# elasota/ConvectionKernels

Hardware: AMD Instinct MI355X
Metric: bc7_encode_default_plan_throughput (higher is better)
Workload: dtype f32+u16; 1 GPU; EncodeBC7, BC7EncodingPlan() + Options(), 4096x4096 SplitMix64 random RGBA, seed 2, 1048576 blocks resident in HBM (BASELINE configs[1]); blocks=1048576, exchange=none, search=exact branch-and-bound (output bit-identical)

## Files before the change

### convectionkernels_amd/csrc/bc7_kernel.hip

```cpp
#include <hip/hip_runtime.h>
#include <stdint.h>
#include <float.h>
#include <type_traits>
#include <stdlib.h>

#include "cvtt_device.h"

constexpr int kMaxPTRefine = 2;
constexpr float kBoundGrid16 = 2000.0f, kBoundLimit16 = 2040.0f;
constexpr float kBoundGrid8 = 124.0f, kBoundLimit8 = 127.0f;
#ifndef CVTT_GRID8_RGBA
#define CVTT_GRID8_RGBA true
#endif
#ifndef CVTT_GRID8_RGB
#define CVTT_GRID8_RGB true
#endif
#ifndef CVTT_BC7_WAVES
#define CVTT_BC7_WAVES 4
#endif
#ifndef CVTT_BC7_WAVES_SLOW
#define CVTT_BC7_WAVES_SLOW 4
#endif
#ifndef CVTT_EIG_ITERS
#define CVTT_EIG_ITERS 6
#endif

#include "cvtt_kernel_common.h"

#ifndef CVTT_SPEC_1
#define CVTT_SPEC_1 32
#define CVTT_SPEC_2 16
#define CVTT_SPEC_4 8
#define CVTT_SPEC_8 4
#endif
#ifndef CVTT_SPEC_16
#define CVTT_SPEC_16 2
#endif
#ifndef CVTT_FILTER_STRIKES
#define CVTT_FILTER_STRIKES 2
#endif
#ifndef CVTT_SHARP_COST4
#define CVTT_SHARP_COST4 64
#endif
#ifndef CVTT_SHARP_COST8
#define CVTT_SHARP_COST8 20
#endif
#ifndef CVTT_PEND_MIN
#define CVTT_PEND_MIN 20
#endif

#ifdef CVTT_BC7_PROFILE
__device__ unsigned long long g_bc7Prof[48];
__device__ unsigned long long g_bc7Dup[8];
__device__ unsigned long long g_bc7Stage[6][8];
__device__ unsigned long long g_bc7Stage2[6][8];
extern "C" int cvttmi_bc7_stage_read(unsigned long long *out)
{
    unsigned long long zero[48] = {0};
    if (hipMemcpyFromSymbol(out, HIP_SYMBOL(g_bc7Stage), sizeof(zero)) != hipSuccess) return -1;
    if (hipMemcpyToSymbol(HIP_SYMBOL(g_bc7Stage), zero, sizeof(zero)) != hipSuccess) return -1;
    if (hipMemcpyFromSymbol(out + 48, HIP_SYMBOL(g_bc7Stage2), sizeof(zero)) != hipSuccess) return -1;
    if (hipMemcpyToSymbol(HIP_SYMBOL(g_bc7Stage2), zero, sizeof(zero)) != hipSuccess) return -1;
    return 0;
}
#define PROF_STAGE(stage, slot, n) { const unsigned long long v_ = (unsigned long long)(n); if (threadIdx.x == 0 && v_) atomicAdd(&g_bc7Stage[stage][slot], v_); }
#define PROF_STAGE_LANES(stage, slot, pred) { const unsigned long long v_ = (unsigned long long)__popcll(__ballot(pred)); if (threadIdx.x == 0 && v_) atomicAdd(&g_bc7Stage[stage][slot], v_); }
#define PROF_STAGE2(stage, slot, n) { const unsigned long long v_ = (unsigned long long)(n); if (threadIdx.x == 0 && v_) atomicAdd(&g_bc7Stage2[stage][slot], v_); }
extern "C" int cvttmi_bc7_dup_read(unsigned long long *out)
{
    unsigned long long zero[8] = {0};
    if (hipMemcpyFromSymbol(out, HIP_SYMBOL(g_bc7Dup), sizeof(zero)) != hipSuccess) return -1;
    if (hipMemcpyToSymbol(HIP_SYMBOL(g_bc7Dup), zero, sizeof(zero)) != hipSuccess) return -1;
    return 0;
}
#define PROF_DECL unsigned long long profT = __builtin_readcyclecounter(); unsigned long long profAcc[16] = {0, 0, 0, 0, 0, 0, 0, 0, 0, 0, 0, 0, 0, 0, 0, 0}; unsigned long long profCnt[8] = {0, 0, 0, 0, 0, 0, 0, 0};
#define PROF_MARK(slot) { const unsigned long long now = __builtin_readcyclecounter(); profAcc[slot] += now - profT; profT = now; }
#define PROF_FLUSH if (threadIdx.x == 0) { unsigned long long tot = 0; for (int i = 0; i < 16; i++) { atomicAdd(&g_bc7Prof[i], profAcc[i]); tot += profAcc[i]; } \
    int bucket = 63 - __builtin_clzll(tot | 1ull) - 12; bucket = bucket < 0 ? 0 : (bucket > 15 ? 15 : bucket); atomicAdd(&g_bc7Prof[16 + bucket], 1ull); \
    } { unsigned long long wsum[8]; for (int i = 0; i < 8; i++) { unsigned long long v = profCnt[i]; if (i >= 4) { for (int st = 1; st < 64; st <<= 1) v += __shfl_xor(v, st); } wsum[i] = v; } \
    if (threadIdx.x == 0) { for (int i = 0; i < 8; i++) atomicAdd(&g_bc7Prof[32 + i], wsum[i]); \
    const unsigned long long passes = profCnt[2] / 64ull; int pb = 63 - __builtin_clzll(passes | 1ull); pb = pb > 7 ? 7 : pb; atomicAdd(&g_bc7Prof[40 + pb], 1ull); } }
#define PROF_COUNT(slot, n) { profCnt[slot] += (unsigned long long)(n); }
extern "C" int cvttmi_bc7_prof_read(unsigned long long *out)
{
    unsigned long long zero[48] = {0};
    if (hipMemcpyFromSymbol(out, HIP_SYMBOL(g_bc7Prof), sizeof(zero)) != hipSuccess) return -1;
    if (hipMemcpyToSymbol(HIP_SYMBOL(g_bc7Prof), zero, sizeof(zero)) != hipSuccess) return -1;
    return 0;
}
#else
#define PROF_DECL
#define PROF_MARK(slot)
#define PROF_COUNT(slot, n)
#define PROF_FLUSH
#define PROF_STAGE(stage, slot, n)
#define PROF_STAGE2(stage, slot, n)
#define PROF_STAGE_LANES(stage, slot, pred)
#endif

#ifdef CVTT_BC7_DEBUG
__device__ float g_bc7Dbg[2048];
__device__ unsigned g_bc7DbgBlock = 0xffffffffu;
extern "C" int cvttmi_bc7_debug_set(unsigned block)
{
    return hipMemcpyToSymbol(HIP_SYMBOL(g_bc7DbgBlock), &block, sizeof(block)) == hipSuccess ? 0 : -1;
}
extern "C" int cvttmi_bc7_debug_read(float *out)
{
    return hipMemcpyFromSymbol(out, HIP_SYMBOL(g_bc7Dbg), sizeof(float) * 2048) == hipSuccess ? 0 : -1;
}
#endif

namespace
{
__device__ __forceinline__ int quantizeNoP(int v, int bits) { return ((v << bits) - v + (127 + (1 << (7 - bits)))) >> 8; }
__device__ __forceinline__ int quantizeP(int v, int bits, int p)
{
    const int addend = p ? ((1 << (8 - bits)) - 1) : 255;
    const int q = ((v << (bits + 1)) - v + addend) >> 9;
    return (q << 1) | p;
}
__device__ __forceinline__ int unquantize(int v, int bits)
{
    const int t = v << (8 - bits);
    return t | (t >> bits);
}

struct ModeDesc
{
    int mode;
    int indexBits;
    int numP;
    int quantBits;
    int unquantBits;
};

__device__ __forceinline__ void compressEndpoints(const ModeDesc &md, int (&ep)[2][4], int pIter, bool isRGB)
{
    const int nch = isRGB ? 3 : 4;
#pragma unroll
    for (int j = 0; j < 2; j++)
    {
        const int p = (md.numP == 4) ? ((pIter >> j) & 1) : (pIter & 1);
#pragma unroll
        for (int ch = 0; ch < 4; ch++)
        {
            if (ch < nch)
            {
                int v = ep[j][ch];
                v = (md.numP == 1) ? quantizeNoP(v, md.quantBits) : quantizeP(v, md.quantBits, p);
                if (md.unquantBits)
                    v = unquantize(v, md.unquantBits);
                ep[j][ch] = v;
            }
        }
        if (isRGB)
            ep[j][3] = 255;
    }
}

struct ShapeBest
{
    float err;
    u32 ep0, ep1;
    u32 idxLo, idxHi;
};

__device__ __forceinline__ u32 packEP(const int (&e)[4])
{
    return (u32)e[0] | ((u32)e[1] << 8) | ((u32)e[2] << 16) | ((u32)e[3] << 24);
}

__device__ __forceinline__ void quadArgminBroadcast(ShapeBest &b, int lane)
{
    int who = lane & 3;
    float err = b.err;
// ... 1235 lines not shown
        for (int a = 0; a < 4; a++)
#pragma unroll
            for (int b = 0; b <= a; b++)
                r.p[tri(a, b)] = (int)__builtin_amdgcn_udot4(m[a], P[b][g], (u32)r.p[tri(a, b)], false);
    }
}

__device__ __forceinline__ void rawSumsSub(RawSums &d, const RawSums &a)
{
    d.n -= a.n;
#pragma unroll
    for (int i = 0; i < 4; i++)
        d.s[i] -= a.s[i];
#pragma unroll
    for (int i = 0; i < 10; i++)
        d.p[i] -= a.p[i];
}

template <int N>
__device__ __forceinline__ float subsetBoundFull(const RawSums &r, const float (&w)[4], float delta)
{
    if (r.n < 2)
        return 0.0f;
    const float n = (float)r.n;
    const float inv = __builtin_amdgcn_rcpf(n);
    Moments<N> m;
#pragma unroll
    for (int a = 0; a < N; a++)
#pragma unroll
        for (int b = 0; b <= a; b++)
        {
            const int v = __mul24(r.n, r.p[tri(a, b)]) - __mul24(r.s[a], r.s[b]);
            m.cov[tri(a, b)] = (((float)v * inv) * w[a]) * w[b];
        }
    return shapeErrorLowerBound<N>(m, n, delta);
}

__device__ __forceinline__ void topEigenvector(const float (&M)[10], float (&e)[4])
{
    int k = 0;
    float d = M[tri(0, 0)];
#pragma unroll
    for (int i = 1; i < 4; i++)
        if (M[tri(i, i)] > d)
        {
            d = M[tri(i, i)];
            k = i;
        }
    float v[4];
#pragma unroll
    for (int i = 0; i < 4; i++)
        v[i] = (k == 0) ? M[tri(i, 0)] : (k == 1) ? M[tri(i, 1)] : (k == 2) ? M[tri(i, 2)] : M[tri(i, 3)];
    for (int it = 0; it < CVTT_EIG_ITERS; it++)
    {
        float nv[4];
        float big = 0.0f;
#pragma unroll
        for (int r = 0; r < 4; r++)
        {
            float a = M[tri(r, 0)] * v[0];
#pragma unroll
            for (int c = 1; c < 4; c++)
                a = __fmaf_rn(M[tri(r, c)], v[c], a);
            nv[r] = a;
            big = fmaxf(big, fabsf(a));
        }
        const float sc = (big > 0.0f) ? __builtin_amdgcn_rcpf(big) : 0.0f;
#pragma unroll
        for (int r = 0; r < 4; r++)
            v[r] = nv[r] * sc;
    }
    float len = v[0] * v[0];
#pragma unroll
    for (int i = 1; i < 4; i++)
        len = __fmaf_rn(v[i], v[i], len);
    const bool ok = len > 1e-12f && len < 1e12f;
    const float inv = ok ? __builtin_amdgcn_rsqf(len) : 0.0f;
    e[0] = ok ? v[0] * inv : 1.0f;
#pragma unroll
    for (int i = 1; i < 4; i++)
        e[i] = v[i] * inv;
}

template <int N>
__device__ __forceinline__ float subsetBoundSharp(const u32 *lp, u32 mask, const float (&w)[4], float delta, float wSq, bool fourLevels)
{
    RawSums r;
    {
        asm volatile("" : "+v"(lp));
        u32 px[16], CM[4][4];
#pragma unroll
        for (int i = 0; i < 4; i++)
        {
            const uint4 v = *reinterpret_cast<const uint4 *>(lp + 4 * i);
            px[4 * i + 0] = v.x;
            px[4 * i + 1] = v.y;
            px[4 * i + 2] = v.z;
            px[4 * i + 3] = v.w;
        }
        channelMajor(px, CM);
        maskedRawSumsCM(CM, mask, r);
    }
    if (r.n < 2)
        return 0.0f;
    const float n = (float)r.n;
    const float inv = __builtin_amdgcn_rcpf(n);
    Moments<N> m;
#pragma unroll
    for (int a = 0; a < N; a++)
#pragma unroll
        for (int b = 0; b <= a; b++)
        {
            const int v = __mul24(r.n, r.p[tri(a, b)]) - __mul24(r.s[a], r.s[b]);
            m.cov[tri(a, b)] = (((float)v * inv) * w[a]) * w[b];
        }
    float rTrue;
    const float cur = shapeErrorLowerBound<N>(m, n, delta, &rTrue);
    if (r.n < 3 || !(rTrue >= 0.0f))
        return cur;
    float T = 0.0f;
#pragma unroll
    for (int i = 0; i < N; i++)
        T += m.cov[tri(i, i)];
    float e[4];
    {
        float M[10];
#pragma unroll
        for (int i = 0; i < 10; i++)
            M[i] = (N == 4 || i < 6) ? m.cov[i < N * (N + 1) / 2 ? i : 0] : 0.0f;
        topEigenvector(M, e);
    }
    float L = 0.0f, Sd[N];
#pragma unroll
    for (int a = 0; a < N; a++)
    {
        float acc = 0.0f;
#pragma unroll
        for (int b = 0; b < N; b++)
            acc = __fmaf_rn(m.cov[a >= b ? tri(a, b) : tri(b, a)], e[b], acc);
        Sd[a] = acc;
        L = __fmaf_rn(e[a], acc, L);
    }
    float rho2 = 0.0f, aMax = 0.0f, aSum = 0.0f;
#pragma unroll
    for (int a = 0; a < N; a++)
    {
        const float t = Sd[a] - L * e[a];
        rho2 = __fmaf_rn(t, t, rho2);
        const float ac = fabsf(e[a]) * w[a];
        aMax = fmaxf(aMax, ac);
        aSum += ac;
    }
    const float eta = 1e-5f * T;
    const float Llo = fmaxf(L - eta, 0.0f);
    const float Rlo = fmaxf(T - L - eta, 0.0f);
    const float sqrtRhi = __builtin_amdgcn_sqrtf(fmaxf(T - L, 0.0f) + eta) * 1.000001f;
    const float rhoHi = __builtin_amdgcn_sqrtf(rho2) * 1.000001f + eta;
    const float W2 = wSq * 1.000001f;
    const float md = fmaxf(2.0f * aMax - aSum, 0.0f) * 0.99999f;
    const float perp = __builtin_amdgcn_sqrtf(fmaxf(W2 - md * md, 0.0f)) * 1.000001f;

    float sqrtQ = 0.0f;
    constexpr int kMaxN = 13;
    if (fourLevels && r.n > 4 && r.n <= kMaxN)
    {
        float g[4];
// ... 37 lines not shown
        float D2[kMaxN + 1], D3[kMaxN + 1];
        D2[0] = D3[0] = 0.0f;
        {
            float su = 0.0f, sq = 0.0f;
#pragma unroll
            for (int j = 1; j <= kMaxN; j++)
            {
                su += t[j - 1];
                sq = __fmaf_rn(t[j - 1], t[j - 1], sq);
                D2[j] = D3[j] = __fmaf_rn(-su * su, kRcp[j], sq);
            }
        }
        float fin = D3[kMaxN];
        {
            float su0 = 0.0f, sq0 = 0.0f;
#pragma unroll
            for (int i = 1; i < kMaxN; i++)
            {
                su0 += t[i - 1];
                sq0 = __fmaf_rn(t[i - 1], t[i - 1], sq0);
                const float d1 = __fmaf_rn(-su0 * su0, kRcp[i], sq0);
                const float d2 = D2[i], d3 = D3[i];
                float su = 0.0f, sq = 0.0f;
#pragma unroll
                for (int j = i + 1; j <= kMaxN; j++)
                {
                    su += t[j - 1];
                    sq = __fmaf_rn(t[j - 1], t[j - 1], sq);
                    const float cst = __fmaf_rn(-su * su, kRcp[j - i], sq);
                    D2[j] = fminf(D2[j], d1 + cst);
                    D3[j] = fminf(D3[j], d2 + cst);
                }
                const float m = (float)(cnt - i);
                const float last = __fmaf_rn(-su * su, __builtin_amdgcn_rcpf(m), sq);
                fin = (i < cnt) ? fminf(fin, d3 + last) : fin;
            }
        }
        const float Q = fmaxf(fin - 2e-5f * range * range, 0.0f);
        sqrtQ = fmaxf(__builtin_amdgcn_sqrtf(fmaxf(Q * 0.9999f, 0.0f)) - 2e-3f, 0.0f);
    }

    constexpr int kIntervals = 20;
    constexpr float kB0sq[20] = {0.0f, 0.0001f, 0.0004f, 0.0009f, 0.0016f, 0.003025f, 0.0049f, 0.007225f, 0.01f, 0.015625f, 0.0225f, 0.030625f, 0.04f, 0.0625f, 0.09f, 0.140625f, 0.2025f, 0.3025f, 0.49f, 0.7225f};
    constexpr float kB1sq[20] = {0.0001f, 0.0004f, 0.0009f, 0.0016f, 0.003025f, 0.0049f, 0.007225f, 0.01f, 0.015625f, 0.0225f, 0.030625f, 0.04f, 0.0625f, 0.09f, 0.140625f, 0.2025f, 0.3025f, 0.49f, 0.7225f, 1.0f};
    constexpr float kB1[20] = {0.01f, 0.02f, 0.03f, 0.04f, 0.055f, 0.07f, 0.085f, 0.1f, 0.125f, 0.15f, 0.175f, 0.2f, 0.25f, 0.3f, 0.375f, 0.45f, 0.55f, 0.7f, 0.85f, 1.0f};
    constexpr float kA1[20] = {0.999948f, 0.999798f, 0.9995479f, 0.9991977f, 0.9984844f, 0.997545f, 0.996379f, 0.9949854f, 0.9921548f, 0.988684f, 0.9845665f, 0.9797939f, 0.9682439f, 0.9539373f, 0.927023f, 0.8930268f, 0.835163f, 0.7141414f, 0.5267816f, 0.0f};
    constexpr float kCross[20] = {0.00999952f, 0.01999604f, 0.02998656f, 0.03996807f, 0.05491686f, 0.06982843f, 0.08469255f, 0.09949894f, 0.1240198f, 0.1483032f, 0.1722998f, 0.1959596f, 0.2420619f, 0.2861823f, 0.347635f, 0.4018637f, 0.4593415f, 0.499901f, 0.500001f, 0.4477662f};
    float best = FLT_MAX;
#pragma unroll
    for (int j = 0; j < kIntervals; j++)
    {
        const float e0 = __fmaf_rn(kB0sq[j], Llo - Rlo, Rlo), e1 = __fmaf_rn(kB1sq[j], Llo - Rlo, Rlo);
        float base = fminf(e0, e1) * 0.999999f - 2.0f * kCross[j] * rhoHi;
        base = fmaxf(base, rTrue);
        const float qd = fmaxf(kA1[j] * sqrtQ - kB1[j] * sqrtRhi, 0.0f);
        const float G = __fmaf_rn(qd, qd, base);
        const float inner = fmaxf(kA1[j] * md - kB1[j] * perp, 0.0f);
        const float s2 = 0.25f * (W2 - inner * inner) * 1.000001f;
        float v = 0.0f;
        if (G > 4.0001f * n * s2)
            v = G - 2.0f * __builtin_amdgcn_sqrtf(s2 * n * G) * 1.000001f;
        best = fminf(best, v);
    }
    return fmaxf(cur, best * 0.9999f);
}

__device__ __forceinline__ int dot4s(u32 a, u32 b, int acc) { return __builtin_amdgcn_sdot4((int)a, (int)b, acc, false); }
template <bool G8>
struct Proj2D
{
    u32 U[G8 ? 4 : 8], V[G8 ? 4 : 8];
    int tU, tV, tUU, tVV, tUV;
};

template <bool G8>
__device__ __forceinline__ void makeProjection(const u32 (&pix)[16], const BlockScatter &bs, const CvttBc7Args &A,
                                               bool use4, float scale, Proj2D<G8> &P)
{
    float M[10];
#pragma unroll
    for (int i = 0; i < 10; i++)
        M[i] = (use4 || i < 6) ? bs.S[i] : 0.0f;
    float e1[4], e2[4];
    topEigenvector(M, e1);
    {
        float Me[4];
#pragma unroll
        for (int r = 0; r < 4; r++)
        {
            float a = M[tri(r, 0)] * e1[0];
#pragma unroll
            for (int c = 1; c < 4; c++)
                a = __fmaf_rn(M[tri(r, c)], e1[c], a);
            Me[r] = a;
        }
        float lam = Me[0] * e1[0];
#pragma unroll
        for (int r = 1; r < 4; r++)
            lam = __fmaf_rn(Me[r], e1[r], lam);
#pragma unroll
        for (int r = 0; r < 4; r++)
#pragma unroll
            for (int c = 0; c <= r; c++)
                M[tri(r, c)] = __fmaf_rn(-lam * e1[r], e1[c], M[tri(r, c)]);
    }
    topEigenvector(M, e2);
    {
        float d = e2[0] * e1[0];
#pragma unroll
        for (int i = 1; i < 4; i++)
            d = __fmaf_rn(e2[i], e1[i], d);
        float len = 0.0f;
#pragma unroll
        for (int i = 0; i < 4; i++)
        {
            e2[i] = __fmaf_rn(-d, e1[i], e2[i]);
            len = __fmaf_rn(e2[i], e2[i], len);
        }
        if (!(len > 1e-4f))
        {
            int k = 0;
            float small = fabsf(e1[0]);
#pragma unroll
            for (int i = 1; i < 4; i++)
                if ((use4 || i < 3) && fabsf(e1[i]) < small)
                {
                    small = fabsf(e1[i]);
                    k = i;
                }
            const float ek = (k == 0) ? e1[0] : (k == 1) ? e1[1] : (k == 2) ? e1[2] : e1[3];
            len = 0.0f;
#pragma unroll
            for (int i = 0; i < 4; i++)
            {
                e2[i] = ((i == k) ? 1.0f : 0.0f) - ek * e1[i];
                len = __fmaf_rn(e2[i], e2[i], len);
            }
        }
        const float inv = __builtin_amdgcn_rsqf(len);
#pragma unroll
        for (int i = 0; i < 4; i++)
            e2[i] *= inv;
    }
    if (!use4)
        e1[3] = e2[3] = 0.0f;

    float g1[4], g2[4];
    float o1 = 0.0f, o2 = 0.0f;
#pragma unroll
    for (int ch = 0; ch < 4; ch++)
    {
        g1[ch] = e1[ch] * A.w[ch] * scale;
        g2[ch] = e2[ch] * A.w[ch] * scale;
        o1 = __fmaf_rn(e1[ch] * scale, bs.meanW[ch], o1);
        o2 = __fmaf_rn(e2[ch] * scale, bs.meanW[ch], o2);
    }
    P.tU = P.tV = P.tUU = P.tVV = P.tUV = 0;
    if constexpr (G8)
    {
    int tid = (int)__builtin_amdgcn_mbcnt_hi(~0u, __builtin_amdgcn_mbcnt_lo(~0u, 0u));
    asm volatile("" : "+v"(tid));
    const int c = tid & 3;
    u32 myU = 0, myV = 0;
    {
        u32 ub = 0, vb = 0;
#pragma unroll
        for (int h = 0; h < 4; h++)
        {
            const u32 p0 = pix[h], p1 = pix[4 + h], p2 = pix[8 + h], p3 = pix[12 + h];
            const u32 pk = fetchPixel(c == 0 ? p0 : c == 1 ? p1 : c == 2 ? p2 : p3);
            float fu = -o1, fv = -o2;
#pragma unroll
            for (int ch = 0; ch < 4; ch++)
            {
                const float x = byteF(pk, ch);
                fu = __fmaf_rn(g1[ch], x, fu);
                fv = __fmaf_rn(g2[ch], x, fv);
            }
            fu = fminf(fmaxf(fu, -kBoundLimit8), kBoundLimit8);
            fv = fminf(fmaxf(fv, -kBoundLimit8), kBoundLimit8);
            ub |= ((u32)(int)rintf(fu) & 0xffu) << (8 * h);
            vb |= ((u32)(int)rintf(fv) & 0xffu) << (8 * h);
        }
        myU = ub;
        myV = vb;
    }
    const int quadBase = tid & ~3;
#pragma unroll
    for (int k = 0; k < 4; k++)
// ... 22 lines not shown
#pragma unroll
            for (int ch = 0; ch < 4; ch++)
            {
                const float x = byteF(pk, ch);
                fu = __fmaf_rn(g1[ch], x, fu);
                fv = __fmaf_rn(g2[ch], x, fv);
            }
            fu = fminf(fmaxf(fu, -kBoundLimit16), kBoundLimit16);
            fv = fminf(fmaxf(fv, -kBoundLimit16), kBoundLimit16);
            uu[h] = (int)rintf(fu);
            vv[h] = (int)rintf(fv);
        }
        P.U[k] = ((u32)uu[0] & 0xffffu) | ((u32)uu[1] << 16);
        P.V[k] = ((u32)vv[0] & 0xffffu) | ((u32)vv[1] << 16);
        P.tU = dot2(P.U[k], 0x00010001u, P.tU);
        P.tV = dot2(P.V[k], 0x00010001u, P.tV);
        P.tUU = dot2(P.U[k], P.U[k], P.tUU);
        P.tVV = dot2(P.V[k], P.V[k], P.tVV);
        P.tUV = dot2(P.U[k], P.V[k], P.tUV);
    }
    }
}

struct Sums2D
{
    int n, u, v, uu, vv, uv;
};

__device__ __forceinline__ void maskedSumsSel(const Proj2D<true> &P, int n, const uint4 &sel, Sums2D &m)
{
    m.n = n;
    m.u = m.v = m.uu = m.vv = m.uv = 0;
    const u32 s4[4] = {sel.x, sel.y, sel.z, sel.w};
#pragma unroll
    for (int k = 0; k < 4; k++)
    {
        const u32 um = P.U[k] & s4[k], vm = P.V[k] & s4[k];
        m.u = dot4s(um, 0x01010101u, m.u);
        m.v = dot4s(vm, 0x01010101u, m.v);
        m.uu = dot4s(um, P.U[k], m.uu);
        m.vv = dot4s(vm, P.V[k], m.vv);
        m.uv = dot4s(um, P.V[k], m.uv);
    }
}

template <bool G8>
__device__ __forceinline__ void maskedSums(const Proj2D<G8> &P, u32 mask, Sums2D &m)
{
    m.n = __popc(mask);
    m.u = m.v = m.uu = m.vv = m.uv = 0;
    if constexpr (G8)
    {
#pragma unroll
    for (int k = 0; k < 4; k++)
    {
        const u32 bits = (((mask >> (4 * k)) & 0xfu) * 0x00204081u) & 0x01010101u;
        const u32 sel = (bits << 8) - bits;
        const u32 um = P.U[k] & sel, vm = P.V[k] & sel;
        m.u = dot4s(um, 0x01010101u, m.u);
        m.v = dot4s(vm, 0x01010101u, m.v);
        m.uu = dot4s(um, P.U[k], m.uu);
        m.vv = dot4s(vm, P.V[k], m.vv);
        m.uv = dot4s(um, P.V[k], m.uv);
    }
    }
    else
    {
#pragma unroll
    for (int k = 0; k < 8; k++)
    {
        const u32 lo = (u32)__builtin_amdgcn_sbfe(mask, 2 * k, 1);
        const u32 hi = (u32)__builtin_amdgcn_sbfe(mask, 2 * k + 1, 1);
        const u32 sel = (lo & 0x0000ffffu) | (hi & 0xffff0000u);
        const u32 um = P.U[k] & sel, vm = P.V[k] & sel;
        m.u = dot2(um, 0x00010001u, m.u);
        m.v = dot2(vm, 0x00010001u, m.v);
        m.uu = dot2(um, P.U[k], m.uu);
        m.vv = dot2(vm, P.V[k], m.vv);
        m.uv = dot2(um, P.V[k], m.uv);
    }
    }
}

template <bool G8 = false>
__device__ __forceinline__ float subsetBound2D(const Sums2D &m, float invScaleSq, float delta)
{
    if (m.n < 2)
        return 0.0f;
    const int a = (G8 ? __mul24(m.n, m.uu) : m.n * m.uu) - __mul24(m.u, m.u);
    const int c = (G8 ? __mul24(m.n, m.vv) : m.n * m.vv) - __mul24(m.v, m.v);
    const int b = (G8 ? __mul24(m.n, m.uv) : m.n * m.uv) - __mul24(m.u, m.v);
    const float fa = (float)a, fc = (float)c, fb = (float)b;
    const float half = (fa + fc) * 0.5f;
    const float diff = (fa - fc) * 0.5f;
    const float rad = __builtin_amdgcn_sqrtf(__fmaf_rn(diff, diff, fb * fb));
    const float lam = half * 0.999998f - rad * 1.000002f;
    const float n = (float)m.n;
    const float L = lam * invScaleSq;
    float lb = 0.0f;
    if (L > n * n * delta * delta)
        lb = (L * __builtin_amdgcn_rcpf(n) - 2.0f * delta * __builtin_amdgcn_sqrtf(L)) * 0.9999f;
    return lb > 0.0f ? lb : 0.0f;
}

}

__device__ __forceinline__ u32 everyFourth(u64 m, int c)
{
    u64 x = (m >> c) & 0x1111111111111111ull;
    x = (x | (x >> 3)) & 0x0303030303030303ull;
    x = (x | (x >> 6)) & 0x000f000f000f000full;
    x = (x | (x >> 12)) & 0x000000ff000000ffull;
    x = (x | (x >> 24)) & 0xffffull;
    return (u32)x;
}

template <bool FAST, bool PT, bool HARD>
__device__ __forceinline__ void bc7Body(const uint8_t *__restrict__ blocks, uint8_t *__restrict__ out,
                                        const CvttBc7Args &A, const CvttDeviceTables *__restrict__ T,
                                        const CvttBc7DevicePlan *__restrict__ dplan, const u32 vBlock, const u32 vGrid)
{
    __shared__ unsigned short s_bound[64][16];
    auto lbLoadRaw = [&](int partition, int b) -> float { return __builtin_bit_cast(float, (u32)s_bound[partition][b] << 16); };
    auto lbLoad = [&](int partition, int b) -> float { return __builtin_fabsf(lbLoadRaw(partition, b)); };
    auto lbStore = [&](int partition, int b, float v) { s_bound[partition][b] = (unsigned short)(__builtin_bit_cast(u32, v) >> 16); };
    auto lbStoreTier2 = [&](int partition, int b, float v) { s_bound[partition][b] = (unsigned short)((__builtin_bit_cast(u32, v) >> 16) | 0x8000u); };
    u32 *const s_raw = reinterpret_cast<u32 *>(&s_bound[0][0]);
    __shared__ u32 s_pix[16][16];
    __shared__ u32 s_blkFlags[16];
    __shared__ int s_scatter[16][14];
    __shared__ u32 s_item[64];
    __shared__ uint8_t s_myItems[PT ? 16 : 1][32];
    __shared__ UnitRec s_unit[64];
    __shared__ u32 s_parked[16][2];
    __shared__ float s_static[16];
    __shared__ unsigned short s_pm2[64];
    __shared__ u32 s_pm3[64];
    __shared__ __attribute__((aligned(16))) u32 s_res[64][5];
    __shared__ float s_trialErr[PT ? 32 * 16 * kMaxPTRefine : 1];
    float *const trialHbm = (PT && A.ptTrial) ? A.ptTrial + (size_t)vBlock * (size_t)(32 * 16) * (size_t)(A.refineRounds < 1 ? 1 : A.refineRounds) : nullptr;
    const cvttmi_bc7_plan *__restrict__ plan = &dplan->plan;
    int lane = threadIdx.x;
    int c = lane & 3;
    int blk = lane >> 2;
#define REFRESH_LANE() do { lane = (int)__builtin_amdgcn_mbcnt_hi(~0u, __builtin_amdgcn_mbcnt_lo(~0u, 0u)); asm volatile("" : "+v"(lane)); c = lane & 3; blk = lane >> 2; } while (0)
    u32 hardIndex = 0, hardBlock = 0;
    u64 hardMine = 0;
    float hardErr = FLT_MAX;
    int hardSeq = -1;
    if (HARD)
    {
        hardIndex = vBlock / kHardWaves;
        const u32 count = *A.hardCount;
        if (hardIndex >= (count < A.hardCap ? count : A.hardCap))
            return;
        const CvttBc7HardRec rec = A.hardRec[hardIndex];
        hardBlock = rec.blockIndex;
        hardErr = rec.err;
        hardSeq = rec.seq;
        u64 m = ((u64)rec.aliveHi << 32) | rec.aliveLo;
        const int q = (int)(vBlock % kHardWaves);
        for (int r = 0; m != 0; r++)
        {
            const u64 low = m & (0ull - m);
            if ((r % kHardWaves) == q)
                hardMine |= low;
            m ^= low;
        }
        if (hardMine == 0)
        {
            if (lane == 0)
                A.hardCand[vBlock].err = FLT_MAX;
            return;
        }
    }
    const u32 blockIndex = (HARD ? (hardBlock & ~15u) : vBlock * 16u) + (u32)(lane >> 2);
    const bool inRange = blockIndex < A.numBlocks;
    enum : u32 { LF_VALID = 1u, LF_ANY_ALPHA = 2u, LF_ALLOW_RGB = 4u, LF_ALLOW_M7 = 8u, LF_NONMAX_ALPHA = 16u };
    u32 lf = (inRange && (!HARD || blockIndex == hardBlock)) ? LF_VALID : 0u;
#define valid ((lf & LF_VALID) != 0)
#define anyBlockHasAlpha ((lf & LF_ANY_ALPHA) != 0)
#define allowRGBModes ((lf & LF_ALLOW_RGB) != 0)
#define allowMode7 ((lf & LF_ALLOW_M7) != 0)
#define blockHasNonMaxAlpha ((lf & LF_NONMAX_ALPHA) != 0)

// ... 325 lines not shown
            {
                const int cfgSlot = (int)g_bc7Dbg[0];
                g_bc7Dbg[1 + cfgSlot] = (float)(rotation * 100 + cfg);
                g_bc7Dbg[0] = (float)(cfgSlot + 1);
            }
#endif
            const float combined = b.err + bA.err;
            const int seq = 384 + cfg;
#ifdef CVTT_BC7_PROFILE
            {
                const float lbp = lbRotOf(rotation);
                const bool needed = valid && c == 0 && !(lbp > work.err);
                PROF_COUNT(6, (needed && (bA.err + lbp > work.err)) ? 1 : 0)
                if (needed && simN < 12)
                {
                    simKey[simN] = lbp + bA.err;
                    simErr[simN] = combined;
                    simN++;
                }
            }
#endif
            if (combined < work.err || (combined == work.err && seq < workSeq))
            {
                work.err = combined;
                workSeq = seq;
                const u32 iLo = indexSelector ? bA.idxLo : b.idxLo, iHi = indexSelector ? bA.idxHi : b.idxHi;
                workPay0 = (c == 0) ? (b.ep0 | bA.ep0) : (c == 3) ? iLo : 0u;
                workPay1 = (c == 0) ? (b.ep1 | bA.ep1) : (c == 3) ? iHi : 0u;
                s_parked[lane >> 2][0] = indexSelector ? b.idxLo : bA.idxLo;
                s_parked[lane >> 2][1] = indexSelector ? b.idxHi : bA.idxHi;
            }
        }
#ifdef CVTT_BC7_PROFILE
        {
            float best = FLT_MAX;
            int evald = 0;
            u32 left = (1u << simN) - 1u;
            while (left)
            {
                int pick = -1;
                float pk = FLT_MAX;
                for (int i = 0; i < 12; i++)
                    if (((left >> i) & 1u) && (pick < 0 || simKey[i] < pk))
                    {
                        pick = i;
                        pk = simKey[i];
                    }
                if (pk > best)
                    break;
                evald++;
                best = simErr[pick] < best ? simErr[pick] : best;
                left &= ~(1u << pick);
            }
            PROF_COUNT(7, evald)
        }
#endif
        __syncthreads();
        PROF_MARK(1)
    }

    auto subsetMaskOf = [&](int numSub, int partition, int sub) -> u32 {
        if (numSub == 1)
            return 0xffffu;
        if (numSub == 2)
        {
            const u32 m1 = s_pm2[partition];
            return sub ? m1 : (~m1 & 0xffffu);
        }
        const u32 m = s_pm3[partition];
        const u32 m1 = m & 0xffffu, m2 = m >> 16;
        return sub == 1 ? m1 : sub == 2 ? m2 : (~(m1 | m2) & 0xffffu);
    };
    auto pixFromLds = [&](u32 (&px)[16]) {
#pragma unroll
        for (int i = 0; i < 4; i++)
        {
            const uint4 v = *reinterpret_cast<const uint4 *>(&s_pix[blk][4 * i]);
            px[4 * i + 0] = v.x;
            px[4 * i + 1] = v.y;
            px[4 * i + 2] = v.z;
            px[4 * i + 3] = v.w;
        }
    };
    enum : int { WS_BOUNDS_FOR = 0, WS_BOUND_BITS = 3, WS_SHARP_RAN = 6, WS_SHARP_NOPAY = 9, WS_T2_NOPAY = 12, WS_STRIKES = 15 };
    u32 ws = (4u << WS_BOUND_BITS) | (4u << WS_SHARP_RAN);
#define WS_GET(f) ((int)((ws >> (f)) & 7u))
#define WS_SET(f, v) do { ws = (u32)__builtin_amdgcn_readfirstlane((int)((ws & ~(7u << (f))) | ((u32)(v) << (f)))); } while (0)
    if (c == 0)
        s_static[blk] = 0.0f;
    if (prune)
    {
        u32 acc = 0;
        u32 lpix[16];
        pixFromLds(lpix);
#pragma unroll
        for (int px = 0; px < 16; px++)
        {
            const int d = 255 - byteI(lpix[px], 3);
            acc = (u32)mad24(d, d, (int)acc);
        }
        if (c == 0)
            s_static[blk] = ((A.flags & CVTTMI_FLAG_UNIFORM) ? (float)(int)acc : (float)(int)acc * A.wSq[3]) * 0.9999f;
    }

    for (int stageOrder = 0; stageOrder < 6; stageOrder++)
    {
        REFRESH_LANE();
        const int stageIter = (ballotA == 0 && !HARD) ? ((stageOrder == 1) ? 2 : (stageOrder == 2) ? 3 : (stageOrder == 3) ? 1 : stageOrder) : stageOrder;
        ModeDesc md;
        int numSubsets, numPartitions, stage, boundSet;
        switch (stageIter)
        {
        case 0: stage = 4; md = {6, 4, 4, 7, 0}; numSubsets = 1; numPartitions = 1; boundSet = 3; break;
        case 1: stage = 5; md = {7, 2, 4, 5, 6}; numSubsets = 2; numPartitions = 64; boundSet = 0; break;
        case 2: stage = 1; md = {1, 3, 2, 6, 7}; numSubsets = 2; numPartitions = 64; boundSet = 1; break;
        case 3: stage = 3; md = {3, 2, 4, 7, 0}; numSubsets = 2; numPartitions = 64; boundSet = 1; break;
        case 4: stage = 0; md = {0, 3, 4, 4, 5}; numSubsets = 3; numPartitions = 16; boundSet = 2; break;
        default: stage = 2; md = {2, 2, 1, 5, 5}; numSubsets = 3; numPartitions = 64; boundSet = 2; break;
        }
        if (HARD && stageIter != 1)
            continue;
        if (stageIter == 1 && ballotA == 0)
            boundSet = 1;
        const int mode = md.mode;
        const bool isRGB = mode < 4;
        const bool laneRuns = isRGB ? allowRGBModes : (mode == 7 ? allowMode7 : true);
        if (__ballot(laneRuns) == 0)
            continue;
        u64 enabled;
        switch (stageIter)
        {
        case 0: enabled = plan->mode6Enabled ? 1 : 0; break;
        case 1: enabled = ~0ull; break;
        case 2: enabled = plan->mode1PartitionEnabled; break;
        case 3: enabled = plan->mode3PartitionEnabled; break;
        case 4: enabled = plan->mode0PartitionEnabled & 0xffffull; break;
        default: enabled = plan->mode2PartitionEnabled; break;
        }
        if (HARD)
            enabled = hardMine;
        if (enabled == 0)
            continue;

        u32 freshAlive = 0;
        bool freshBounds = false;
        if (prune)
        {
            if (WS_GET(WS_BOUNDS_FOR) == boundSet + 1 && WS_GET(WS_BOUND_BITS) < md.indexBits)
                WS_SET(WS_BOUNDS_FOR, 0);
            if (WS_GET(WS_BOUNDS_FOR) != boundSet + 1)
            {
                WS_SET(WS_BOUND_BITS, 4);
                WS_SET(WS_SHARP_RAN, 4);
                __syncthreads();
                if (boundSet == 3)
                {
                }
                else
                {
                    const bool use4 = (boundSet == 0);
                    auto boundsOnGrid = [&](auto g8) {
                    constexpr bool G8 = decltype(g8)::value;
                    const float wsum = A.wSqSum3 + (use4 ? A.wSq[3] : 0.0f);
                    const float scale = (G8 ? kBoundGrid8 : kBoundGrid16) / (255.0f * __builtin_amdgcn_sqrtf(wsum));
                    const float invScaleSq = 1.0f / (scale * scale);
                    const float delta = (use4 ? A.delta4 : A.delta3) + 0.7072f / scale;
                    Proj2D<G8> P;
                    PROF_MARK(2)
                    {
                        BlockScatter bsL;
                        {
                            int rs[4], rp[10];
#pragma unroll
                            for (int i = 0; i < 10; i++)
                                rp[i] = s_scatter[blk][i];
#pragma unroll
                            for (int i = 0; i < 4; i++)
                                rs[i] = s_scatter[blk][10 + i];
                            scatterFromRaw(rs, rp, A, bsL);
                        }
                        u32 lpix[16];
                        pixFromLds(lpix);
                        makeProjection(lpix, bsL, A, use4, scale, P);
                    }
                    PROF_MARK(7)
                    const bool two = boundSet < 2;
                    auto selOf = [&](int partition, int which) -> uint4 {
                        return *reinterpret_cast<const uint4 *>(T->subsetByteMask[two ? partition : 64 + 2 * partition + which]);
                    };
                    uint4 selA = make_uint4(0, 0, 0, 0), selB = make_uint4(0, 0, 0, 0);
                    if constexpr (G8)
                    {
                        selA = selOf(c, 0);
                        if (!two)
                            selB = selOf(c, 1);
                    }
                    for (int k = 0; k < 16; k++)
                    {
                        const int partition = 4 * k + c;
                        float lb;
                        uint4 selA1 = selA, selB1 = selB;
                        if constexpr (G8)
                        {
                            const int nextPartition = (k < 15 ? partition + 4 : partition);
                            selA1 = selOf(nextPartition, 0);
                            if (!two)
                                selB1 = selOf(nextPartition, 1);
                        }
                        if (boundSet < 2)
                        {
                            Sums2D s1, s0;
                            if constexpr (G8)
                                maskedSumsSel(P, __popc((u32)s_pm2[partition]), selA, s1);
                            else
                                maskedSums(P, s_pm2[partition], s1);
                            s0.n = 16 - s1.n;
                            s0.u = P.tU - s1.u;
                            s0.v = P.tV - s1.v;
                            s0.uu = P.tUU - s1.uu;
                            s0.vv = P.tVV - s1.vv;
                            s0.uv = P.tUV - s1.uv;
                            lb = subsetBound2D<G8>(s0, invScaleSq, delta) + subsetBound2D<G8>(s1, invScaleSq, delta);
                        }
                        else
                        {
                            Sums2D s1, s2, s0;
                            if constexpr (G8)
                            {
                                maskedSumsSel(P, __popc(s_pm3[partition] & 0xffffu), selA, s1);
                                maskedSumsSel(P, __popc(s_pm3[partition] >> 16), selB, s2);
                            }
                            else
                            {
                            maskedSums(P, s_pm3[partition] & 0xffffu, s1);
                            maskedSums(P, s_pm3[partition] >> 16, s2);
                            }
                            s0.n = 16 - s1.n - s2.n;
                            s0.u = P.tU - s1.u - s2.u;
                            s0.v = P.tV - s1.v - s2.v;
                            s0.uu = P.tUU - s1.uu - s2.uu;
                            s0.vv = P.tVV - s1.vv - s2.vv;
                            s0.uv = P.tUV - s1.uv - s2.uv;
                            lb = subsetBound2D<G8>(s0, invScaleSq, delta) + subsetBound2D<G8>(s1, invScaleSq, delta) +
                                 subsetBound2D<G8>(s2, invScaleSq, delta);
                        }
                        if (!use4)
                            lb += s_static[blk];
                        lbStore(partition, blk, lb);
                        freshAlive |= (lb > work.err) ? 0u : (1u << k);
                        selA = selA1;
                        selB = selB1;
                    }
                    freshBounds = true;
                    };
                    if (use4 ? CVTT_GRID8_RGBA : CVTT_GRID8_RGB)
                        boundsOnGrid(std::true_type{});
                    else
                        boundsOnGrid(std::false_type{});
                }
                __syncthreads();
                WS_SET(WS_BOUNDS_FOR, boundSet + 1);
            }
        }
        PROF_MARK(2)

        const int CP = md.numP * 4;
        const int UPB = 64 / CP;
        u32 aliveBits = (valid && laneRuns) ? everyFourth(enabled, c) : 0u;
        if (mode == 7 && anyBlockHasAlpha && !blockHasNonMaxAlpha)
            aliveBits &= everyFourth(mode7RGB, c);
        u32 tier2Done = 0;
        if (prune)
        {
            if (freshBounds)
                aliveBits &= freshAlive;
            else
            {
                for (int k = 0; k * 4 < numPartitions; k++)
                {
// ... 1368 lines not shown
```

Measured before the change: 687.2 Mblocks/s.

## Add tier-0 cheap partition rejection with LDS compaction queue and quad-parallel eigenvectors

Adds a cheap tier-0 test on two-subset partitions that rules out a partition from its 2D moments without the sqrt-based bound. Surviving candidates are compacted into an LDS queue and evaluated densely across the wave. This is meant to cut divergent per-lane bound work. The power-iteration eigenvector is also split across a lane quad with DPP permutes, which reduces per-lane FMA work. Both add __syncthreads, borrow shared buffers, and carry a self-disable heuristic when too many partitions stay open.

```diff
diff --git a/convectionkernels_amd/csrc/bc7_kernel.hip b/convectionkernels_amd/csrc/bc7_kernel.hip
--- a/convectionkernels_amd/csrc/bc7_kernel.hip
+++ b/convectionkernels_amd/csrc/bc7_kernel.hip
@@ -24,6 +24,14 @@
 #ifndef CVTT_EIG_ITERS
 #define CVTT_EIG_ITERS 6
 #endif
+#ifndef CVTT_TIER0
+#define CVTT_TIER0 1
+#endif
+#ifndef CVTT_TIER0_THETA
+#define CVTT_TIER0_THETA 0.0625f
+#endif
+constexpr float kTier0Theta = CVTT_TIER0_THETA;
+constexpr int kTier0Slots = 64, kTier0Fields = 8;
 
 #include "cvtt_kernel_common.h"
 
@@ -81,6 +89,7 @@
     if (threadIdx.x == 0) { for (int i = 0; i < 8; i++) atomicAdd(&g_bc7Prof[32 + i], wsum[i]); \
     const unsigned long long passes = profCnt[2] / 64ull; int pb = 63 - __builtin_clzll(passes | 1ull); pb = pb > 7 ? 7 : pb; atomicAdd(&g_bc7Prof[40 + pb], 1ull); } }
 #define PROF_COUNT(slot, n) { profCnt[slot] += (unsigned long long)(n); }
+#define PROF_TIER0(slot, n) { profAcc[8 + (slot)] += (unsigned long long)(n); }
 extern "C" int cvttmi_bc7_prof_read(unsigned long long *out)
 {
     unsigned long long zero[48] = {0};
@@ -92,6 +101,7 @@
 #define PROF_DECL
 #define PROF_MARK(slot)
 #define PROF_COUNT(slot, n)
+#define PROF_TIER0(slot, n)
 #define PROF_FLUSH
 #define PROF_STAGE(stage, slot, n)
 #define PROF_STAGE2(stage, slot, n)
@@ -1493,6 +1503,56 @@
         e[i] = v[i] * inv;
 }
 
+template <int QUAD_PERM>
+__device__ __forceinline__ float quadPerm(float v)
+{
+    return __int_as_float(__builtin_amdgcn_mov_dpp(__float_as_int(v), QUAD_PERM, 0xf, 0xf, true));
+}
+
+#ifndef CVTT_EIG_QUAD
+#define CVTT_EIG_QUAD 1
+#endif
+__device__ __forceinline__ void topEigenvectorQuad(const float (&M)[10], int c, float (&e)[4])
+{
+    int k = 0;
+    float d = M[tri(0, 0)];
+#pragma unroll
+    for (int i = 1; i < 4; i++)
+        if (M[tri(i, i)] > d)
+        {
+            d = M[tri(i, i)];
+            k = i;
+        }
+    float row[4];
+#pragma unroll
+    for (int j = 0; j < 4; j++)
+        row[j] = (c == 0) ? M[tri(0, j)] : (c == 1) ? M[tri(1, j)] : (c == 2) ? M[tri(2, j)] : M[tri(3, j)];
+    float mine = (k == 0) ? row[0] : (k == 1) ? row[1] : (k == 2) ? row[2] : row[3];
+    for (int it = 0; it < CVTT_EIG_ITERS; it++)
+    {
+        float a = row[0] * quadPerm<0x00>(mine);
+        a = __fmaf_rn(row[1], quadPerm<0x55>(mine), a);
+        a = __fmaf_rn(row[2], quadPerm<0xaa>(mine), a);
+        a = __fmaf_rn(row[3], quadPerm<0xff>(mine), a);
+        float big = fabsf(a);
+        big = fmaxf(big, quadPerm<0xb1>(big));
+        big = fmaxf(big, quadPerm<0x4e>(big));
+        const float sc = (big > 0.0f) ? __builtin_amdgcn_rcpf(big) : 0.0f;
+        mine = a * sc;
+    }
+    const float v[4] = {quadPerm<0x00>(mine), quadPerm<0x55>(mine), quadPerm<0xaa>(mine), quadPerm<0xff>(mine)};
+    float len = v[0] * v[0];
+#pragma unroll
+    for (int i = 1; i < 4; i++)
+        len = __fmaf_rn(v[i], v[i], len);
+    const bool ok = len > 1e-12f && len < 1e12f;
+    const float inv = ok ? __builtin_amdgcn_rsqf(len) : 0.0f;
+    e[0] = ok ? v[0] * inv : 1.0f;
+#pragma unroll
+    for (int i = 1; i < 4; i++)
+        e[i] = v[i] * inv;
+}
+
 template <int N>
 __device__ __forceinline__ float subsetBoundSharp(const u32 *lp, u32 mask, const float (&w)[4], float delta, float wSq, bool fourLevels)
 {
@@ -1696,7 +1756,12 @@
     for (int i = 0; i < 10; i++)
         M[i] = (use4 || i < 6) ? bs.S[i] : 0.0f;
     float e1[4], e2[4];
-    topEigenvector(M, e1);
+    int quadLane = (int)__builtin_amdgcn_mbcnt_lo(~0u, 0u) & 3;
+    asm volatile("" : "+v"(quadLane));
+    if (CVTT_EIG_QUAD)
+        topEigenvectorQuad(M, quadLane, e1);
+    else
+        topEigenvector(M, e1);
     {
         float Me[4];
 #pragma unroll
@@ -1718,7 +1783,10 @@
             for (int c = 0; c <= r; c++)
                 M[tri(r, c)] = __fmaf_rn(-lam * e1[r], e1[c], M[tri(r, c)]);
     }
-    topEigenvector(M, e2);
+    if (CVTT_EIG_QUAD)
+        topEigenvectorQuad(M, quadLane, e2);
+    else
+        topEigenvector(M, e2);
     {
         float d = e2[0] * e1[0];
 #pragma unroll
@@ -1907,25 +1975,57 @@
     }
 }
 
+struct Moments2D
+{
+    int a, b, c;
+};
+
 template <bool G8 = false>
-__device__ __forceinline__ float subsetBound2D(const Sums2D &m, float invScaleSq, float delta)
-{
-    if (m.n < 2)
+__device__ __forceinline__ void subsetMoments2D(const Sums2D &m, Moments2D &q)
+{
+    q.a = (G8 ? __mul24(m.n, m.uu) : m.n * m.uu) - __mul24(m.u, m.u);
+    q.c = (G8 ? __mul24(m.n, m.vv) : m.n * m.vv) - __mul24(m.v, m.v);
+    q.b = (G8 ? __mul24(m.n, m.uv) : m.n * m.uv) - __mul24(m.u, m.v);
+}
+
+__device__ __forceinline__ float subsetBound2DTail(const Moments2D &q, int count, float invScaleSq, float delta)
+{
+    if (count < 2)
         return 0.0f;
-    const int a = (G8 ? __mul24(m.n, m.uu) : m.n * m.uu) - __mul24(m.u, m.u);
-    const int c = (G8 ? __mul24(m.n, m.vv) : m.n * m.vv) - __mul24(m.v, m.v);
-    const int b = (G8 ? __mul24(m.n, m.uv) : m.n * m.uv) - __mul24(m.u, m.v);
-    const float fa = (float)a, fc = (float)c, fb = (float)b;
+    const float fa = (float)q.a, fc = (float)q.c, fb = (float)q.b;
     const float half = (fa + fc) * 0.5f;
     const float diff = (fa - fc) * 0.5f;
     const float rad = __builtin_amdgcn_sqrtf(__fmaf_rn(diff, diff, fb * fb));
     const float lam = half * 0.999998f - rad * 1.000002f;
-    const float n = (float)m.n;
+    const float n = (float)count;
     const float L = lam * invScaleSq;
     float lb = 0.0f;
     if (L > n * n * delta * delta)
         lb = (L * __builtin_amdgcn_rcpf(n) - 2.0f * delta * __builtin_amdgcn_sqrtf(L)) * 0.9999f;
     return lb > 0.0f ? lb : 0.0f;
+}
+
+template <bool G8 = false>
+__device__ __forceinline__ float subsetBound2D(const Sums2D &m, float invScaleSq, float delta)
+{
+    if (m.n < 2)
+        return 0.0f;
+    Moments2D q;
+    subsetMoments2D<G8>(m, q);
+    return subsetBound2DTail(q, m.n, invScaleSq, delta);
+}
+
+__device__ __forceinline__ bool tier0RulesOut(const Moments2D &q0, const Moments2D &q1, float n1, float K)
+{
+    const float a0 = (float)q0.a, b0 = (float)q0.b, c0 = (float)q0.c;
+    const float a1 = (float)q1.a, b1 = (float)q1.b, c1 = (float)q1.c;
+    const float n0 = 16.0f - n1;
+    const float e0 = a0 - c0, e1 = a1 - c1;
+    const float rho0 = __fmaf_rn(4.0f * b0, b0, e0 * e0), rho1 = __fmaf_rn(4.0f * b1, b1, e1 * e1);
+    const float pos = __fmaf_rn(n0, a1 + c1, n1 * (a0 + c0));
+    const float Z = __fmaf_rn(pos, 0.99999f, -((2.0f * K) * (n0 * n1)));
+    const float rhs = __fmaf_rn(n0 * n0, rho1, (n1 * n1) * rho0);
+    return Z > 0.0f && Z * Z > 2.001f * rhs;
 }
 
 }
@@ -2417,7 +2517,7 @@
             px[4 * i + 3] = v.w;
         }
     };
-    enum : int { WS_BOUNDS_FOR = 0, WS_BOUND_BITS = 3, WS_SHARP_RAN = 6, WS_SHARP_NOPAY = 9, WS_T2_NOPAY = 12, WS_STRIKES = 15 };
+    enum : int { WS_BOUNDS_FOR = 0, WS_BOUND_BITS = 3, WS_SHARP_RAN = 6, WS_SHARP_NOPAY = 9, WS_T2_NOPAY = 12, WS_STRIKES = 15, WS_T0_NOPAY = 18 };
     u32 ws = (4u << WS_BOUND_BITS) | (4u << WS_SHARP_RAN);
 #define WS_GET(f) ((int)((ws >> (f)) & 7u))
 #define WS_SET(f, v) do { ws = (u32)__builtin_amdgcn_readfirstlane((int)((ws & ~(7u << (f))) | ((u32)(v) << (f)))); } while (0)
@@ -2530,6 +2630,101 @@
                         if (!two)
                             selB = selOf(c, 1);
                     }
+                    bool tier0 = false;
+                    if constexpr (G8)
+                        tier0 = CVTT_TIER0 && two && WS_GET(WS_T0_NOPAY) == 0;
+                    if (tier0)
+                    {
+                        if constexpr (G8)
+                        {
+                        const float settled = __fmaf_rn(work.err, 1.01f, 1e-20f);
+                        const float K = ((settled * 1.0002f + (16.001f / kTier0Theta) * (delta * delta)) * (scale * scale)) * (1.0001f / (1.0f - kTier0Theta));
+                        static_assert(sizeof(s_unit) >= sizeof(u32) * kTier0Fields * kTier0Slots && sizeof(s_res) >= sizeof(u32) * 64, "tier 0 borrows s_unit and s_res");
+                        u32 *const queue = reinterpret_cast<u32 *>(&s_unit[0]);
+                        u32 *const aliveWord = &s_res[0][0];
+                        aliveWord[lane] = 0;
+                        int queued = 0;
+                        for (int k = 0; k < 16; k++)
+                        {
+                            const int partition = 4 * k + c;
+                            const uint4 selA1 = selOf(k < 15 ? partition + 4 : partition, 0);
+                            const int n1 = __popc((u32)s_pm2[partition]);
+                            Sums2D s1, s0;
+                            maskedSumsSel(P, n1, selA, s1);
+                            s0.n = 16 - s1.n;
+                            s0.u = P.tU - s1.u;
+                            s0.v = P.tV - s1.v;
+                            s0.uu = P.tUU - s1.uu;
+                            s0.vv = P.tVV - s1.vv;
+                            s0.uv = P.tUV - s1.uv;
+                            Moments2D q0, q1;
+                            subsetMoments2D<true>(s0, q0);
+                            subsetMoments2D<true>(s1, q1);
+                            const bool open = valid && !tier0RulesOut(q0, q1, (float)n1, K);
+                            const u64 openMask = __ballot(open);
+                            if (open)
+                            {
+                                const int slot = queued + (int)__builtin_amdgcn_mbcnt_hi((u32)(openMask >> 32), __builtin_amdgcn_mbcnt_lo((u32)openMask, 0u));
+                                if (slot < kTier0Slots)
+                                {
+                                    queue[0 * kTier0Slots + slot] = (u32)q0.a;
+                                    queue[1 * kTier0Slots + slot] = (u32)q0.b;
+                                    queue[2 * kTier0Slots + slot] = (u32)q0.c;
+                                    queue[3 * kTier0Slots + slot] = (u32)q1.a;
+                                    queue[4 * kTier0Slots + slot] = (u32)q1.b;
+                                    queue[5 * kTier0Slots + slot] = (u32)q1.c;
+                                    queue[6 * kTier0Slots + slot] = (u32)partition | ((u32)lane << 8) | ((u32)n1 << 16);
+                                    queue[7 * kTier0Slots + slot] = __builtin_bit_cast(u32, work.err);
+                                }
+                                else
+                                {
+                                    float lb = subsetBound2DTail(q0, 16 - n1, invScaleSq, delta) + subsetBound2DTail(q1, n1, invScaleSq, delta);
+                                    if (!use4)
+                                        lb += s_static[blk];
+                                    lbStore(partition, blk, lb);
+                                    freshAlive |= (lb > work.err) ? 0u : (1u << k);
+                                }
+                            }
+                            else
+                                lbStore(partition, blk, settled);
+                            queued += __popcll(openMask);
+                            selA = selA1;
+                        }
+                        PROF_TIER0(0, queued)
+                        PROF_TIER0(2, 1)
+                        __syncthreads();
+                        const int inQueue = queued < kTier0Slots ? queued : kTier0Slots;
+                        for (int base = 0; base < inQueue; base += 64)
+                        {
+                            PROF_TIER0(1, 1)
+                            const int slot = base + lane;
+                            if (slot < inQueue)
+                            {
+                                Moments2D q0, q1;
+                                q0.a = (int)queue[0 * kTier0Slots + slot];
+                                q0.b = (int)queue[1 * kTier0Slots + slot];
+                                q0.c = (int)queue[2 * kTier0Slots + slot];
+                                q1.a = (int)queue[3 * kTier0Slots + slot];
+                                q1.b = (int)queue[4 * kTier0Slots + slot];
+                                q1.c = (int)queue[5 * kTier0Slots + slot];
+                                const u32 what = queue[6 * kTier0Slots + slot];
+                                const float ownerErr = __builtin_bit_cast(float, queue[7 * kTier0Slots + slot]);
+                                const int partition = (int)(what & 0xffu), owner = (int)((what >> 8) & 0xffu), n1 = (int)(what >> 16);
+                                float lb = subsetBound2DTail(q0, 16 - n1, invScaleSq, delta) + subsetBound2DTail(q1, n1, invScaleSq, delta);
+                                if (!use4)
+                                    lb += s_static[owner >> 2];
+                                lbStore(partition, owner >> 2, lb);
+                                if (!(lb > ownerErr))
+                                    atomicOr(&aliveWord[owner], 1u << (partition >> 2));
+                            }
+                        }
+                        __syncthreads();
+                        freshAlive |= aliveWord[lane];
+                        if (2 * queued > 16 * __popcll(__ballot(valid)))
+                            WS_SET(WS_T0_NOPAY, 1);
+                        }
+                    }
+                    else
                     for (int k = 0; k < 16; k++)
                     {
                         const int partition = 4 * k + c;
```

Result: slower. 514.4 Mblocks/s (-25.1%).
